# revdotcom/paper_accurate_fast_cheap

Hardware: AMD Instinct MI355X
Metric: audio-sec/sec (1/RTF) GigaSpeech long-form encode (higher is better)
Workload: dtype f32+bf16-slot

## Files before the change

include/pafc_encoder_ops.h:

```cpp
#ifndef PAFC_ENCODER_OPS_H
#define PAFC_ENCODER_OPS_H

#include "pafc_wkv6.h"

#ifdef __cplusplus
extern "C" {
#endif

int pafc_dwconv1d_cl(int dtype, int B, int T_in, int C, int K, int left_pad, int T_out, const void *x,
                     const void *w, const void *bias, void *y, int glu, const int32_t *lens,
                     pafc_stream_t stream);

int pafc_dwconv1d_cl_ex(int dtype, int B, int T_in, int C, int K, int left_pad, int T_out, const void *x, long ldx,
                        const void *w, const void *bias, void *y, int act, const int32_t *lens, pafc_stream_t stream);

int pafc_dwconv1d_cl_ln_silu(int dtype, int B, int T_in, int C, int K, int left_pad, int T_out, const void *x, long ldx,
                             const void *w, const void *bias, const void *gamma, const void *beta, float eps, void *y,
                             const int32_t *lens, pafc_stream_t stream);

size_t pafc_dwconv1d_cl_wgrad_workspace_bytes(int B, int T_out, int C, int K);
int pafc_dwconv1d_cl_wgrad(int dtype, int B, int T_in, int C, int K, int left_pad, int T_out, const void *x, long ldx,
                           const void *dy, float *dw, float *dbias, void *workspace, size_t workspace_bytes,
                           pafc_stream_t stream);

// ... 148 lines not shown

int pafc_mamba2_scan_skip_bf16(int B, int L, int H, const void *xbc, long ldx, const float *dt, const float *log_a,
                               const float *D, void *y_bf16, int reverse, int chunk_len, void *workspace,
                               size_t workspace_bytes, pafc_stream_t stream);
int pafc_mamba2_gate_norm(int dtype, long rows, int d_inner, const void *y, const void *z, long ld_z,
                          const void *norm_weight, float eps, void *out, pafc_stream_t stream);

int pafc_mamba2_scan_state(int B, int L, int H, const void *xbc, long ldx, const float *dt, const float *log_a, const float *D,
                           float *y_f32, void *y_bf16, const float *s_in, float *s_out, int reverse, int chunk_len,
                           void *workspace, size_t workspace_bytes, pafc_stream_t stream);

size_t pafc_mamba2_scan_bwd_workspace_bytes(int B, int L, int H, int chunk_len);
int pafc_mamba2_scan_backward(int B, int L, int H, const void *xbc, long ldx, const float *dt, const float *log_a,
                              const float *gy, void *g_xbc, long ldg, float *g_dt, float *g_la, int reverse, int chunk_len,
                              void *workspace, size_t workspace_bytes, pafc_stream_t stream);

int pafc_gemm_bf16(long M, int N, int K, int batch, const void *A, long lda, long strideA, const void *W, long ldw,
                   long strideW, const void *bias, long strideBias, const void *residual, long ldr, long strideR,
                   void *out, long ldo, long strideO, float alpha, int act, pafc_stream_t stream);
int pafc_gemm_bf16_glu_half(long M, int N, int K, int batch);
int pafc_conv3x3s2_nhwc_bf16_ph(int B, int T1, int F1, int Ci, int Co, const void *in, const void *w_tap_co_ci, const void *bias,
                                void *out, int relu, int tile_m, pafc_stream_t stream);
int pafc_gemm_bf16_ph(long M, int N, int K, int batch, const void *A, long lda, long strideA, const void *W, long ldw,
                      long strideW, const void *bias, long strideBias, const void *residual, long ldr, long strideR,
                      void *out, long ldo, long strideO, float alpha, int act, int tile_n, int tile_m, pafc_stream_t stream);
int pafc_gemm_ph_ex(long M, int N, int K, int batch, const void *A, long lda, long strideA, int a_split, const void *W, long ldw,
                    long strideW, const void *bias, long strideBias, const void *residual, int res_kind, long ldr, long strideR,
                    void *out, int out_kind, long ldo, long lo_off, long strideO, float alpha, int act, int tile_m,
                    pafc_stream_t stream);
int pafc_gemm_ph_ex2(long M, int N, int K, int batch, const void *A, long lda, long strideA, int a_split, int a_plane_block,
                     const void *W, long ldw, long strideW, const void *bias, long strideBias, const void *residual, int res_kind,
                     long ldr, long strideR, void *out, int out_kind, long ldo, long lo_off, long strideO, float alpha, int act,
                     int tile_m, pafc_stream_t stream);
int pafc_conv3x3s2_nhwc_split_ph(int B, int T1, int F1, int Ci, int Co, const void *in_planes, const void *w3_tap_co_3ci,
                                 const float *bias, void *out_planes, int relu, int tile_m, pafc_stream_t stream);

int pafc_residual_dropout(int backward, int dtype_x, int dtype_y, long n, const void *x, const void *y, void *out, float scale,
                          float p, unsigned long long seed, unsigned long long offset, pafc_stream_t stream);
int pafc_silu_dropout(int backward, int dtype, long n, const void *h, const void *dout, void *out, float p,
                      unsigned long long seed, unsigned long long offset, pafc_stream_t stream);

int pafc_multi_transpose_bf16(const void *table, int n, int total_tiles, pafc_stream_t stream);
int pafc_multi_cast_bf16(const void *table, int n, int total_chunks, pafc_stream_t stream);

int pafc_rows_gather(const long *table, const long *table_dev, int n, const int *idx, const int *offs, int m, int S,
                     pafc_stream_t stream);
int pafc_rows_scatter(const long *table, const long *table_dev, int n, const int *idx, int m, int S, pafc_stream_t stream);

#ifdef __cplusplus
}
#endif
#endif
```

paper_accurate_fast_cheap_amd/_lib.py:

```python
import ctypes
import os
from ctypes import c_float, c_int, c_long, c_size_t, c_ulonglong, c_void_p

import torch

_HERE = os.path.dirname(os.path.abspath(__file__))
SO_PATH = os.path.join(_HERE, "libpafc_hip.so")

PAFC_F32, PAFC_BF16 = 0, 1
_ERRORS = {
    -1: "null pointer", -2: "bad dims (B, T, C, H must be positive and C == H * 64)", -3: "head size must be 64",
    -4: "workspace too small", -5: "kernel launch failed", -6: "unsupported dtype", -7: "unsupported",
    -8: "r, k, v, w, y must be 16-byte aligned",
}


class PafcError(RuntimeError):
    pass


_lib = None


def lib():
# ... 60 lines not shown
    "pafc_conv3x3s2_nhwc_f32split": (I, [I, I, I, I, I, P, P, P, P, P, P, I, P]),
    "pafc_gemm_tn_workspace_bytes": (Z, [G, I, I]),
    "pafc_gemm_tn_bf16": (I, [G, I, I, P, G, P, G, P, P, I, P, Z, P]),
    "pafc_gemm_tn_batched_workspace_bytes": (Z, [G, I, I, I]),
    "pafc_gemm_tn_bf16_batched": (I, [G, I, I, I, P, G, G, P, G, G, P, P, I, P, Z, P]),
    "pafc_gemm_bf16_f32out": (I, [G, I, I, P, G, I, P, G, P, P, G, P, I, G, G, F, I, P, Z, P]),
    "pafc_gemm_bf16_f32out_pb": (I, [G, I, I, P, G, I, I, P, G, P, P, G, P, I, G, G, F, I, P, Z, P]),
    "pafc_gemm_bf16_f32out_workspace_bytes": (Z, [G, I, I, I]),
    "pafc_ctc_loss_workspace_bytes": (Z, [I, I, I]),
    "pafc_ctc_loss_forward": (I, [I, I, I, I, P, G, P, P, I, P, I, I, P, P, Z, P]),
    "pafc_ctc_loss_backward": (I, [I, I, I, I, P, G, P, P, I, P, I, I, P, P, F, P, G, P, Z, P]),
    "pafc_rnnt_joint_loss_workspace_bytes": (Z, [I, I, I, G, G, P, I]),
    "pafc_rnnt_joint_loss_forward": (I, [I, I, I, I, I, P, G, G, P, G, G, P, P, P, P, P, I, I, G, P, P, Z, P]),
    "pafc_rnnt_joint_loss_backward": (I, [I, I, I, I, I, P, G, G, P, G, G, P, P, P, P, P, I, I, G, P, G, P, F, I, P, P, P, P,
        P, Z, P, Z, P]),
    "pafc_gemm_f32": (I, [G, I, I, I, P, G, G, P, G, G, P, G, P, G, G, P, G, G, F, I, P]),
    "pafc_mamba2_prep": (I, [I, I, I, I, P, P, G, P, P, P, P, P, P, P, P, P]),
    "pafc_mamba2_finish": (I, [I, I, I, I, P, P, P, P, G, P, G, P, P, P, F, I, P, P]),
    "pafc_mamba2_scan_chunk_len": (I, [I, I, I]),
    "pafc_mamba2_scan_workspace_bytes": (Z, [I, I, I, I]),
    "pafc_mamba2_scan": (I, [I, I, I, P, G, P, P, P, I, P, Z, P]),
    "pafc_mamba2_scan_dir": (I, [I, I, I, P, G, P, P, P, I, I, P, Z, P]),
    "pafc_mamba2_scan_skip_bf16": (I, [I, I, I, P, G, P, P, P, P, I, I, P, Z, P]),
    "pafc_mamba2_gate_norm": (I, [I, G, I, P, P, G, P, F, P, P]),
    "pafc_mamba2_scan_state": (I, [I, I, I, P, G, P, P, P, P, P, P, P, I, I, P, Z, P]),
    "pafc_mamba2_scan_bwd_workspace_bytes": (Z, [I, I, I, I]),
    "pafc_mamba2_scan_backward": (I, [I, I, I, P, G, P, P, P, P, G, P, P, I, I, P, Z, P]),
    "pafc_gemm_bf16": (I, [G, I, I, I, P, G, G, P, G, G, P, G, P, G, G, P, G, G, F, I, P]),
    "pafc_gemm_bf16_glu_half": (I, [G, I, I, I]),
    "pafc_conv3x3s2_nhwc_bf16_ph": (I, [I, I, I, I, I, P, P, P, P, I, I, P]),
    "pafc_gemm_bf16_ph": (I, [G, I, I, I, P, G, G, P, G, G, P, G, P, G, G, P, G, G, F, I, I, I, P]),
    "pafc_gemm_ph_ex": (I, [G, I, I, I, P, G, G, I, P, G, G, P, G, P, I, G, G, P, I, G, G, G, F, I, I, P]),
    "pafc_gemm_ph_ex2": (I, [G, I, I, I, P, G, G, I, I, P, G, G, P, G, P, I, G, G, P, I, G, G, G, F, I, I, P]),
    "pafc_conv3x3s2_nhwc_split_ph": (I, [I, I, I, I, I, P, P, P, P, I, I, P]),
    "pafc_residual_dropout": (I, [I, I, I, G, P, P, P, F, F, U, U, P]),
    "pafc_silu_dropout": (I, [I, I, G, P, P, P, F, U, U, P]),
    "pafc_multi_transpose_bf16": (I, [P, I, I, P]),
    "pafc_multi_cast_bf16": (I, [P, I, I, P]),
    "pafc_rows_gather": (I, [P, P, I, P, P, I, I, P]),
    "pafc_rows_scatter": (I, [P, P, I, P, I, I, P]),
    "pafc_fbank_num_frames": (G, [G]),
    "pafc_fbank_tables_cols": (I, []),
    "pafc_fbank_f32": (I, [P, G, P, P, P, P, P, I, P, F, F, P, P]),
    "pafc_fbank_batch": (I, [P, G, P, I, G, P, P, P, P, P, I, P, F, F, P, I, P, P]),
    "pafc_fbank_stream_plan": (I, [I, G, P, P]),
    "pafc_fbank_stream": (I, [P, I, P, G, G, I, P, P, P, P, P, I, F, F, P, I, G, G, P]),
    "pafc_fbank_stream_rows": (I, [P, I, P, P, I, P, G, G, P, P, P, P, P, I, F, F, P, I, I, P]),
    "pafc_ctc_greedy": (I, [I, I, I, I, P, P, I, P, P, P, P, P]),
    "pafc_log_softmax_rows": (I, [I, G, I, P, P, P]),
    "pafc_ctc_prefix_beam_workspace_bytes": (Z, [I, I, I]),
    "pafc_ctc_prefix_beam_search": (I, [I, I, I, P, P, P, I, I, P, P, P, P, Z, P]),
    "pafc_ctc_prefix_beam_ex_workspace_bytes": (Z, [I, I, I]),
    "pafc_ctc_prefix_beam_search_ex": (I, [I, I, I, P, P, P, I, I, P, P, P, P, P, P, Z, P]),
    "pafc_ctc_beam_stream_workspace_bytes": (Z, [I, I, I, I]),
    "pafc_ctc_beam_stream_reset": (I, [I, I, I, I, P, P, Z, P]),
    "pafc_ctc_beam_stream_feed": (I, [I, I, I, P, P, P, I, I, I, P, I, P, Z, P]),
    "pafc_ctc_beam_stream_drain": (I, [I, I, I, P, I, P, Z, P, I, P, P, P, P, P, P, I, P, P, P]),
    "pafc_ctc_greedy_stream_workspace_bytes": (Z, [I]),
    "pafc_ctc_greedy_stream_reset": (I, [I, P, P, Z, P]),
    "pafc_ctc_greedy_stream": (I, [I, I, I, I, P, P, I, P, Z, P, P, P, P, P]),
    "pafc_ctc_align_workspace_bytes": (Z, [I, I, I]),
    "pafc_ctc_align": (I, [I, I, I, I, P, G, P, P, I, P, I, P, Z, P, P, P, I, P, P, P]),
    "pafc_rnnt_beam_workspace_bytes": (Z, [I, I, I]),
    "pafc_rnnt_beam_init": (I, [I, I, I, I, P, Z, P, P, P]),
    "pafc_rnnt_beam_step": (I, [I, I, I, I, I, P, P, P, P, P, Z, P, P, P]),
    "pafc_rnnt_beam_finish": (I, [I, I, I, P, Z, P, P, P, P]),
# ... 79 lines not shown
```

paper_accurate_fast_cheap_amd/csrc/gemm_bf16.hip:

```cpp
#include <stdio.h>
#include <stdlib.h>

#include "pafc_common.h"
#include "../../include/pafc_encoder_ops.h"

namespace pafc {
namespace {

constexpr int GBM = 128, GBN = 128, GBK = 64;
typedef float f32x4g __attribute__((ext_vector_type(4)));
typedef __bf16 bf16x8g __attribute__((ext_vector_type(8)));

struct GemmParams {
    const bf16_t *A, *W, *bias, *res;
    bf16_t *out;
    long M;
    int N, K;
    long lda, ldw, ldo, ldr;
    long sA, sW, sO, sB, sR;
    float alpha;
    int act;
    int mtiles, ntiles;
    int nk1, K1;
    int pb_sh;
// ... 294 lines not shown
                *reinterpret_cast<uint4 *>(Oz + m * p.ldo + n0 + c8) = *reinterpret_cast<const uint4 *>(O + row * LDO + c8);
        }
    }
}

}
}

extern "C" int pafc_gemm_bf16_ph(long M, int N, int K, int batch, const void *A, long lda, long strideA, const void *W, long ldw,
                                 long strideW, const void *bias, long strideBias, const void *residual, long ldr, long strideR,
                                 void *out, long ldo, long strideO, float alpha, int act, int tile_n, int tile_m,
                                 pafc_stream_t stream);

static int ph_tile_m(long M, int N, int K, int batch, int act, bool has_residual) {
    if (N % 8 || K % 128 || N < 256) return 0;
    if (act == 4 && N % 256) return 0;
    if (has_residual && act != 0) return 0;
    const int cus = pafc::device_cus();
    const long nt = (N + 255) / 256;
    static const long min_fill = [] { const char *e = getenv("PAFC_PH_MIN_FILL"); return e ? atol(e) : 0L; }();
    if (min_fill > 0) {
        if (((M + 255) / 256) * nt * batch * 100 < (long)cus * min_fill) return 0;
    } else if (((M + 127) / 128) * ((N + 127) / 128) * batch <= 2L * cus) {
        return 0;
    }
    long best_cost = -1;
    int best = 0;
    for (int tm = 256; tm >= 192; tm -= 64) {
        const long tiles = ((M + tm - 1) / tm) * nt * batch;
        const long cost = ((tiles + cus - 1) / cus) * (tm + 64);
        if (best_cost < 0 || cost < best_cost) { best_cost = cost; best = tm; }
    }
    return best;
}

extern "C" int pafc_gemm_bf16_glu_half(long M, int N, int K, int batch) { return ph_tile_m(M, N, K, batch, 4, false) ? 32 : 64; }

extern "C" int pafc_gemm_bf16(long M, int N, int K, int batch, const void *A, long lda, long strideA, const void *W,
                              long ldw, long strideW, const void *bias, long strideBias, const void *residual, long ldr,
                              long strideR, void *out, long ldo, long strideO, float alpha, int act,
                              pafc_stream_t stream) {
    if (!A || !W || !out) return PAFC_ERR_NULL_POINTER;
    if (M <= 0 || N <= 0 || K <= 0 || batch <= 0 || batch > 65535) return PAFC_ERR_BAD_DIMS;
    if (N % 8 || K % pafc::GBK) return PAFC_ERR_UNSUPPORTED;
    if (act < 0 || act > 4) return PAFC_ERR_UNSUPPORTED;
    if (const int tm = ph_tile_m(M, N, K, batch, act, residual != nullptr)) {
        const int rc = pafc_gemm_bf16_ph(M, N, K, batch, A, lda, strideA, W, ldw, strideW, bias, strideBias, residual, ldr, strideR,
                                         out, ldo, strideO, alpha, act, 256, tm, stream);
        if (rc != PAFC_ERR_UNSUPPORTED) return rc;
        if (act == 4) return PAFC_ERR_UNSUPPORTED;
    }
    const bool glu = act == 4;
    if (glu && (N % pafc::GBN || residual)) return PAFC_ERR_UNSUPPORTED;
    if (lda < K || ldw < K || ldo < (glu ? N / 2 : N) || (residual && ldr < N)) return PAFC_ERR_BAD_DIMS;
    if ((lda | ldw | ldo | strideA | strideW | strideO) % 8 || (residual && ((ldr | strideR) % 8))) return PAFC_ERR_ALIGNMENT;
    if ((((uintptr_t)A | (uintptr_t)W | (uintptr_t)out | (uintptr_t)residual) & 15) != 0) return PAFC_ERR_ALIGNMENT;
    pafc::GemmParams p{};
    p.A = (const pafc::bf16_t *)A; p.W = (const pafc::bf16_t *)W; p.bias = (const pafc::bf16_t *)bias;
    p.res = (const pafc::bf16_t *)residual; p.out = (pafc::bf16_t *)out;
    p.M = M; p.N = N; p.K = K;
    p.lda = lda; p.ldw = ldw; p.ldo = ldo; p.ldr = ldr;
    p.sA = strideA; p.sW = strideW; p.sO = strideO; p.sB = strideBias; p.sR = strideR;
    p.alpha = alpha; p.act = act;
    const long cus = pafc::device_cus();
    auto tiles = [&](int bm, int bn) { return ((M + bm - 1) / bm) * ((N + bn - 1) / bn) * (long)batch; };
    int bm = 128, bn = 128;
// ... 190 lines not shown
```

paper_accurate_fast_cheap_amd/csrc/gemm_ph.hip:

```cpp
#include <climits>
#include <cstdlib>
#include <cstring>
#include <type_traits>

#include "pafc_common.h"
#include "../../include/pafc_encoder_ops.h"

namespace pafc {
namespace {

typedef float f32x4p __attribute__((ext_vector_type(4)));
typedef __bf16 bf16x8p __attribute__((ext_vector_type(8)));
typedef unsigned u32x4p __attribute__((ext_vector_type(4)));

struct PhParams {
    const bf16_t *A, *W;
    const void *bias;
    const void *res;
    void *out;
    long M;
    int N, K;
    long lda, ldw, ldo, ldr;
    long sA, sW, sO, sB, sR;
    float alpha;
// ... 26 lines not shown
                                             uniform_off, 0, 0);
}
__device__ __forceinline__ __amdgpu_buffer_rsrc_t make_rsrc(const void *base, long bytes) {
    return __builtin_amdgcn_make_buffer_rsrc(const_cast<void *>(base), 0, (int)(bytes > 0x7fffffffL ? 0x7fffffffL : bytes), 0x00020000);
}

typedef float f32x2p __attribute__((ext_vector_type(2)));
typedef __bf16 bf16x2p __attribute__((ext_vector_type(2)));
__device__ __forceinline__ uint32_t pack_bf16(float lo, float hi) {
    return __builtin_bit_cast(uint32_t, __builtin_convertvector(f32x2p{lo, hi}, bf16x2p));
}

template <int ACT>
__device__ __forceinline__ float act_apply(float v) {
    if constexpr (ACT == 1) return v * __builtin_amdgcn_rcpf(1.f + __expf(-v));
    if constexpr (ACT == 2) return 1.f - 2.f * __builtin_amdgcn_rcpf(__expf(2.f * v) + 1.f);
    if constexpr (ACT == 3) return fmaxf(v, 0.f);
    return v;
}

#ifndef PH_ST_AUX
#define PH_ST_AUX 0
#endif
#define PH_WAIT(N) asm volatile("s_waitcnt vmcnt(" #N ")" ::: "memory")
template <int N>
__device__ __forceinline__ void wait_vm() {
    static_assert(N >= 0 && N < 64, "vmcnt is a 6-bit counter");
    asm volatile("s_waitcnt vmcnt(%0)" ::"n"(N) : "memory");
}

constexpr int PBN = 256, PBK = 64;
constexpr unsigned PH_OOB = 0xC0000000u;

template <bool GLU, int ACT, int RES, int OUT, bool CONV = false, int LNF = 0, bool SPL = false>
__global__ __launch_bounds__(512, 2) void gemm_ph_kernel(const PhParams p) {
    constexpr int BN = PBN;
    constexpr int UA = 128 * 128;
    constexpr int UB = (BN / 2) * 128;
    constexpr int STEP = 2 * UA + 2 * UB;
    constexpr int OFF_A0 = 0, OFF_A1 = UA, OFF_B0 = 2 * UA, OFF_B1 = 2 * UA + UB;
    constexpr int TN = 2;
    constexpr int DA = UA / 8192;
    constexpr int DB = UB / 8192;
    constexpr int OSZ = OUT == 1 ? 4 : 2;
    constexpr bool BIASF32 = OUT != 0;
    constexpr int NST = 8 * (GLU ? 1 : 2) * (OUT == 0 ? 1 : 2) + (LNF == 2 ? 8 : 0);
    static_assert(LNF == 0 || (OUT == 0 && !CONV), "LayerNorm folding: bf16 GEMMs");
    static_assert(!SPL || LNF == 0, "shared-fragment split operands: not with a folded LayerNorm");
    static_assert(LNF != 1 || (RES == 0 && (GLU || ACT == 1)), "LNF 1: the w_1 (SiLU) / pointwise_conv1 (GLU) projections");
    static_assert(LNF != 2 || RES == 1, "LNF 2: a residual GEMM");
    static_assert(!(GLU && (ACT != 0 || RES != 0)), "GLU excludes an activation and a residual");
    static_assert(!(RES != 0 && ACT != 0), "the layer never pairs a residual with an activation");
    extern __shared__ __attribute__((aligned(1024))) unsigned char lds[];

    const int tid = threadIdx.x, lane = tid & 63;
    const int wave = __builtin_amdgcn_readfirstlane(tid >> 6);
    const int wr = wave >> 2, wc = wave & 3;
    const long nblk = (long)p.mtiles * p.ntiles;
    const long total = nblk * p.batch;
    const long per = total / 8;
    const int nt = SPL ? p.nsteps : p.K / PBK;

    auto pix_off = [&](long m) -> long {
        const long tf = (long)p.T2 * p.F2;
        const long bb = m / tf, rem = m - bb * tf;
        const long t2 = rem / p.F2, f2 = rem - t2 * p.F2;
        return (((bb * p.T1 + 2 * t2) * p.F1 + 2 * f2) * p.CiA) * 2;
    };

    struct Tile {
        long m0;
        int n0, z, vr;
        __amdgpu_buffer_rsrc_t Ar, Wr;
    };
    auto make_tile = [&](long t, Tile &T) {
        const bool real = t < total;
        long tt = real ? t : 0;
        if (tt < per * 8) tt = (tt % 8) * per + tt / 8;
        T.z = (int)(tt / nblk);
        const long bid = tt % nblk;
        const int mt0 = (int)(bid / p.ntiles), nt0 = (int)(bid % p.ntiles);
        T.m0 = (long)mt0 * p.tm;
        T.n0 = nt0 * BN;
        T.vr = (int)min((long)p.tm, p.M - T.m0);
        if constexpr (CONV) {
// ... 34 lines not shown
                const unsigned coff = SPL ? (unsigned)(16 * (sc & 3) + (sc >> 2) * p.w_lo) : (unsigned)(16 * sc);
                b_off[h][j] = (unsigned)((long)((u >> 5) * 64 + h * 32 + pc) * (CONV ? p.CiW : p.ldw) * 2) + coff;
            }
    };
    auto a_soff = [&](int kt) -> unsigned {
        if constexpr (SPL && !CONV) {
            const int blk = kt >> p.pb_shift, c = kt - (blk << p.pb_shift);
            return (unsigned)(blk * 2 * p.pb_bytes + c * 64);
        } else if constexpr (SPL) {
            const int tap = (kt * p.inv_spt) >> 16, kc = kt - tap * p.spt;
            const int dt = (tap * 11) >> 5, df = tap - 3 * dt;
            return (unsigned)(((dt * p.F1 + df) * p.CiA) * 2 + kc * 64);
        } else if constexpr (!CONV) {
            const int seg = (kt >= p.nk1) + (kt >= 2 * p.nk1);
            const int r = kt - seg * p.nk1;
            const int blk = r >> p.pb_shift, c = r - (blk << p.pb_shift);
            return (unsigned)(blk * 2 * p.pb_bytes + (seg == 1 ? p.pb_bytes : 0) + c * 128);
        } else {
            const int tap = (kt * p.inv_spt) >> 16, kc = kt - tap * p.spt;
            const int seg = (kc >= p.nk1) + (kc >= 2 * p.nk1), cc = kc - seg * p.nk1;
            const int dt = (tap * 11) >> 5, df = tap - 3 * dt;
            return (unsigned)(((dt * p.F1 + df) * p.CiA + (seg == 1 ? p.Ci : 0)) * 2 + cc * 128);
        }
    };
    auto w_soff = [&](int kt) -> unsigned {
        if constexpr (!CONV) return SPL ? kt * p.w_step : kt * 128;
        const int tap = (kt * p.inv_spt) >> 16, kc = kt - tap * p.spt;
        return (unsigned)(tap * p.N * p.CiW * 2 + kc * (SPL ? 64 : 128));
    };
    auto stage_a = [&](const Tile &T, int h, int buf, int kt) {
#ifdef PH_ABL_NODMA
        return;
#endif
#pragma unroll
        for (int j = 0; j < DA; ++j)
            dma16(T.Ar, a_off[h][j], a_soff(kt), lds + buf * STEP + (h ? OFF_A1 : OFF_A0) + (wave * DA + j) * 1024);
    };
    auto stage_b = [&](const Tile &T, int h, int buf, int kt) {
#ifdef PH_ABL_NODMA
        return;
#endif
#pragma unroll
        for (int j = 0; j < DB; ++j)
            dma16(T.Wr, b_off[h][j], w_soff(kt), lds + buf * STEP + (h ? OFF_B1 : OFF_B0) + (wave * DB + j) * 1024);
    };

    const int fr = lane & 15, kq = lane >> 4;
    const unsigned frag = fr * 128 + ((kq ^ (fr & 7)) * 16);
    const unsigned la = wr * (64 * 128) + frag;
    const unsigned lb = wc * (32 * 128) + frag;

    bf16x8p af[4][2], bf0[TN][2], bf1[TN][2];
    auto read_a = [&](int h, int buf) {
#ifdef PH_ABL_NOREAD
        return;
#endif
        const unsigned char *base = lds + buf * STEP + (h ? OFF_A1 : OFF_A0);
#pragma unroll
        for (int i = 0; i < 4; ++i) {
            af[i][0] = *reinterpret_cast<const bf16x8p *>(base + la + i * 2048);
            af[i][1] = *reinterpret_cast<const bf16x8p *>(base + (la ^ 64) + i * 2048);
        }
    };
    auto read_b = [&](int h, int buf, bf16x8p (&dst)[TN][2]) {
#ifdef PH_ABL_NOREAD
        return;
#endif
        const unsigned char *base = lds + buf * STEP + (h ? OFF_B1 : OFF_B0);
#pragma unroll
        for (int j = 0; j < TN; ++j) {
            dst[j][0] = *reinterpret_cast<const bf16x8p *>(base + lb + j * 2048);
            dst[j][1] = *reinterpret_cast<const bf16x8p *>(base + (lb ^ 64) + j * 2048);
        }
    };
// ... 341 lines not shown
                        }
                    }
                    store8(o, live, row, col);
                }
                if constexpr (LNF == 2) { gst1[LNF == 2 ? g : 0] = live ? st1 : 0.f; gst2[LNF == 2 ? g : 0] = live ? st2 : 0.f; }
            }
            if constexpr (LNF == 1) row_norm(vn, nx_rstd, nx_nm);
        }
    }
    if constexpr (LNF == 2) {
        __builtin_amdgcn_sched_barrier(0);
#pragma unroll
        for (int g = 0; g < 8; ++g) { gst1[g] += __shfl_xor(gst1[g], 16, 64); gst2[g] += __shfl_xor(gst2[g], 16, 64); }
#pragma unroll
        for (int g = 0; g < 8; ++g) { gst1[g] += __shfl_xor(gst1[g], 32, 64); gst2[g] += __shfl_xor(gst2[g], 32, 64); }
        typedef unsigned u32x2p __attribute__((ext_vector_type(2)));
#pragma unroll
        for (int g = 0; g < 8; ++g) {
            const int row = wr * 128 + g * 16 + efr;
            const bool ok = ekq == 0 && row < cur.vr;
            const unsigned off = ok ? (unsigned)(row * 64 + ((cur.n0 >> 8) * 4 + wc) * 8) : PH_OOB;
            __builtin_amdgcn_raw_buffer_store_b64(u32x2p{__float_as_uint(gst1[g]), __float_as_uint(gst2[g])}, Sr, off, 0, 0);
        }
    }
    __builtin_amdgcn_sched_barrier(0);
    first = false;
    if constexpr (CONV) make_tile(t + gridDim.x, cur);
    else cur = nxt;
    PH_STAMP(53);
    }
    PH_WAIT(0);
}

template <bool GLU, int ACT, int RES, int OUT, bool CONV = false, int LNF = 0, bool SPL = false>
int launch_ph(const PhParams &p, int batch, hipStream_t s) {
    constexpr size_t lds = 2 * (2 * 128 * 128 + 2 * (PBN / 2) * 128) + 8 * 1024 + (LNF == 1 ? 8 * 1024 + 16 * 1024 : 0);
    auto kern = gemm_ph_kernel<GLU, ACT, RES, OUT, CONV, LNF, SPL>;
    static bool attr_set[64];
    int dev = 0;
    if (hipGetDevice(&dev) != hipSuccess) return PAFC_ERR_LAUNCH;
    if (dev < 0 || dev >= 64 || !attr_set[dev]) {
        if (hipFuncSetAttribute((const void *)kern, hipFuncAttributeMaxDynamicSharedMemorySize, (int)lds) != hipSuccess)
            return PAFC_ERR_LAUNCH;
        if (dev >= 0 && dev < 64) attr_set[dev] = true;
    }
    const int cus = device_cus();
    PhParams q = p;
    q.batch = batch;
    const long total = (long)p.mtiles * p.ntiles * batch;
    const long grid = total < cus ? total : cus;
    hipLaunchKernelGGL(kern, dim3((unsigned)grid), dim3(512), lds, s, q);
    return hipGetLastError() == hipSuccess ? PAFC_OK : PAFC_ERR_LAUNCH;
}

int g_split_walk = -1;
bool split_shared_fragments() {
    if (g_split_walk < 0) {
        const char *e = getenv("PAFC_SPLIT_WALK");
        g_split_walk = !(e && std::strcmp(e, "hilohi") == 0);
    }
    return g_split_walk != 0;
}

}
}

extern "C" int pafc_gemm_ph_ex(long M, int N, int K, int batch, const void *A, long lda, long strideA, int a_split, const void *W,
                               long ldw, long strideW, const void *bias, long strideBias, const void *residual, int res_kind,
                               long ldr, long strideR, void *out, int out_kind, long ldo, long lo_off, long strideO, float alpha,
                               int act, int tile_m, pafc_stream_t stream) {
// ... 156 lines not shown
    p.spt = p.CiW / 64;
    p.inv_spt = (65536 + p.spt - 1) / p.spt;
    for (int kt = 0; kt < p.K / 64 + 2; ++kt)
        if (((kt * p.inv_spt) >> 16) != kt / p.spt) return PAFC_ERR_UNSUPPORTED;
    p.T1 = T1; p.F1 = F1; p.T2 = T2; p.F2 = F2;
    p.in_bytes = (long)B * T1 * F1 * p.CiA * 2;
    p.tm = tile_m;
    p.mtiles = (int)((M + tile_m - 1) / tile_m);
    p.ntiles = (Co + 255) / 256;
    hipStream_t s = (hipStream_t)stream;
    if (split && pafc::split_shared_fragments()) {
        p.spt = Ci / 32;
        p.inv_spt = (65536 + p.spt - 1) / p.spt;
        p.nsteps = 9 * p.spt;
        for (int kt = 0; kt < p.nsteps + 2; ++kt)
            if (((kt * p.inv_spt) >> 16) != kt / p.spt) return PAFC_ERR_UNSUPPORTED;
        p.a_lo = Ci * 2;
        p.w_lo = 2 * Ci * 2;
        return relu ? pafc::launch_ph<false, 3, 0, 2, true, 0, true>(p, 1, s) : pafc::launch_ph<false, 0, 0, 2, true, 0, true>(p, 1, s);
    }
    if (split) return relu ? pafc::launch_ph<false, 3, 0, 2, true>(p, 1, s) : pafc::launch_ph<false, 0, 0, 2, true>(p, 1, s);
    return relu ? pafc::launch_ph<false, 3, 0, 0, true>(p, 1, s) : pafc::launch_ph<false, 0, 0, 0, true>(p, 1, s);
}

extern "C" int pafc_conv3x3s2_nhwc_bf16_ph(int B, int T1, int F1, int Ci, int Co, const void *in, const void *w_tap_co_ci,
                                           const void *bias, void *out, int relu, int tile_m, pafc_stream_t stream) {
    return conv_ph_launch(B, T1, F1, Ci, Co, in, w_tap_co_ci, bias, out, relu, tile_m, 0, stream);
}

extern "C" int pafc_conv3x3s2_nhwc_split_ph(int B, int T1, int F1, int Ci, int Co, const void *in_planes, const void *w3_tap_co_3ci,
                                            const float *bias, void *out_planes, int relu, int tile_m, pafc_stream_t stream) {
    return conv_ph_launch(B, T1, F1, Ci, Co, in_planes, w3_tap_co_3ci, bias, out_planes, relu, tile_m, 1, stream);
}
```

paper_accurate_fast_cheap_amd/hip_ops.py:

```python
import contextlib
import ctypes
import math
import os
import threading
import weakref
from typing import List, Optional

import torch

from . import _lib
from ._lib import c_int, c_void_p
from .utils import graph_step


DISPATCH = dict(skinny_max_rows=640, own_gemm_min_rows=1, lds_resident_min_rows=8192, split_gemm_min_rows=1024,
                ln_fold_min_rows=24576, dwconv_ln_silu_max_rows=24575, split_small_max_rows=8192, split_layers_min_rows=256)


def _load_dispatch():
    legacy = dict(skinny_max_rows="PAFC_SKINNY_MAX_ROWS", own_gemm_min_rows="PAFC_OWN_GEMM_MIN_ROWS",
                  lds_resident_min_rows="PAFC_LDS_RESIDENT_MIN_ROWS", split_gemm_min_rows="PAFC_SPLIT_GEMM_MIN_ROWS")
    for name, env in legacy.items():
        if os.environ.get(env):
            DISPATCH[name] = int(os.environ[env])
    for item in filter(None, os.environ.get("PAFC_DISPATCH", "").split(",")):
        name, _, value = item.partition("=")
        if name.strip() not in DISPATCH:
            raise ValueError(f"PAFC_DISPATCH: unknown threshold {name!r} (known: {sorted(DISPATCH)})")
        DISPATCH[name.strip()] = int(value)


_load_dispatch()


def train_gemms_own() -> bool:
    return os.environ.get("PAFC_TRAIN_OWN_GEMMS", "1") != "0"


def train_kernels_enabled() -> bool:
    import os
    return os.environ.get("PAFC_TRAIN_KERNELS", "1") != "0"


def depthwise_conv1d_cl(x: torch.Tensor, weight: torch.Tensor, bias: Optional[torch.Tensor], left_pad: int,
                        out_len: int, glu: bool = False, lens: Optional[torch.Tensor] = None) -> torch.Tensor:
    _lib.require_gpu(x, weight, bias, lens)
    B, T, Cx = x.shape
    C = Cx // 2 if glu else Cx
    K = weight.shape[-1]
# ... 1348 lines not shown
                                    int(ln_c or (K if csum is not None else N)),
                                    float(eps), _ph_tile_m(M, N, min_tm=128), _lib.stream_of(a))
    _lib.check(rc, "pafc_gemm_bf16_ph_ln")
    return out


def split_planes(x: torch.Tensor, triple: bool = False) -> torch.Tensor:
    _lib.require_gpu(x)
    if x.dtype != torch.float32 or x.stride(-1) != 1:
        raise _lib.PafcError("split_planes: contiguous fp32 input")
    K = x.shape[-1]
    rows = x.numel() // K
    out = torch.empty(x.shape[:-1] + ((3 if triple else 2) * K,), dtype=torch.bfloat16, device=x.device)
    L = _lib.lib()
    _lib.check(L.pafc_split_planes(rows, K, _lib.ptr(x), K, _lib.ptr(out), out.shape[-1], K, int(triple), _lib.stream_of(x)),
               "pafc_split_planes")
    return out


def _ph_tile_m(M: int, N: int, batch: int = 1, min_tm: int = 64) -> int:
    cus = torch.cuda.get_device_properties(torch.cuda.current_device()).multi_processor_count
    nt = (N + 255) // 256
    best = None
    for tm in (256, 192, 128, 64):
        if tm < min_tm:
            continue
        tiles = ((M + tm - 1) // tm) * nt * batch
        cost = ((tiles + cus - 1) // cus) * (tm + 64)
        if best is None or cost < best[0]:
            best = (cost, tm)
    return best[1]


def gemm_ph_ex(a: torch.Tensor, w: torch.Tensor, bias: Optional[torch.Tensor] = None, act: str = "none", alpha: float = 1.0,
               residual: Optional[torch.Tensor] = None, out: Optional[torch.Tensor] = None, a_split: bool = False,
               out_kind: str = "bf16", tile_m: int = 0, a_plane_block: int = 0) -> torch.Tensor:
    _lib.require_gpu(bias)
    for t in (a, w, residual, out):
        if t is not None and (not t.is_cuda or t.stride(-1) != 1):
            raise _lib.PafcError("gemm_ph_ex: GPU tensors with unit stride in the last dimension")
    if a.dtype != torch.bfloat16 or w.dtype != torch.bfloat16 or a.dim() != 2 or w.dim() != 2:
        raise _lib.PafcError("gemm_ph_ex: a and w are 2-d bf16 (planes of fp32 operands with a_split)")
    M = a.shape[0]
    N = w.shape[0]
    K = w.shape[1] // 3 if a_split else w.shape[1]
    if a.shape[1] != (2 * K if a_split else K) or (a_split and w.shape[1] != 3 * K):
        raise _lib.PafcError("gemm_ph_ex: a (M, K) x w (N, K); split: a (M, 2K) x w (N, 3K)")
    No = N // 2 if act == "glu" else N
    kinds = {"bf16": (0, torch.bfloat16, No), "f32": (1, torch.float32, No), "planes": (2, torch.bfloat16, 2 * No)}
    ok, odt, ocols = kinds[out_kind]
    if out is None:
        out = torch.empty((M, ocols), dtype=odt, device=a.device)
    if out.dtype != odt or tuple(out.shape) != (M, ocols):
        raise _lib.PafcError("gemm_ph_ex: out must be (M, N) in the output form's dtype ((M, 2N) bf16 for planes)")
    rk = 0
    if residual is not None:
        rk = 1 if residual.dtype == torch.bfloat16 else 2
        if tuple(residual.shape) != (M, N) or residual.dtype != (torch.bfloat16 if ok == 0 else torch.float32) or ok == 2:
            raise _lib.PafcError("gemm_ph_ex: residual (M, N) in the output dtype (bf16 / fp32), not with planes")
    if bias is not None and (bias.dtype != (torch.bfloat16 if ok == 0 else torch.float32) or bias.numel() != N):
        raise _lib.PafcError("gemm_ph_ex: bias (N) bf16 for a bf16 output, fp32 otherwise")
    L = _lib.lib()
    from .profiling import op_timer
    pb_ok = not a_plane_block or (a_split and a_plane_block >= 64 and a_plane_block & (a_plane_block - 1) == 0 and K % a_plane_block == 0)
    if (M <= _SPLIT_SMALL_MAX_ROWS and M * N <= _SPLIT_SMALL_MAX_OUT and ok != 0 and act in ("none", "silu", "tanh", "relu")
            and pb_ok and not tile_m and K % 64 == 0):
        nws = L.pafc_gemm_bf16_f32out_workspace_bytes(M, N, K, int(a_split))
        ws = torch.empty(nws, dtype=torch.uint8, device=a.device) if nws else None
        with op_timer("gemm%ss_%dx%d" % ("3" if a_split else "", K, N), sample=12, flops=2.0 * M * N * K * (3 if a_split else 1)):
            rc = L.pafc_gemm_bf16_f32out_pb(M, N, K, _lib.ptr(a), a.stride(0), int(a_split), int(a_plane_block), _lib.ptr(w), w.stride(0),
                                            _lib.ptr(bias), _lib.ptr(residual), residual.stride(0) if residual is not None else 0,
                                            _lib.ptr(out), ok, out.stride(0), No if ok == 2 else 0, float(alpha), _ACTS[act], _lib.ptr(ws),
                                            nws, _lib.stream_of(a))
        _lib.check(rc, "pafc_gemm_bf16_f32out")
        return out
    with op_timer("gemm%s_%dx%d" % ("3" if a_split else "", K, N), sample=12, flops=2.0 * M * N * K * (3 if a_split else 1)):
        rc = L.pafc_gemm_ph_ex2(M, N, K, 1, _lib.ptr(a), a.stride(0), 0, int(a_split), int(a_plane_block), _lib.ptr(w), w.stride(0), 0,
                                _lib.ptr(bias), 0,
                               _lib.ptr(residual), rk, residual.stride(0) if residual is not None else 0, 0, _lib.ptr(out), ok,
                               out.stride(0), No if ok == 2 else 0, 0, float(alpha), _ACTS[act], int(tile_m or _ph_tile_m(M, N)),
                               _lib.stream_of(a))
    _lib.check(rc, "pafc_gemm_ph_ex")
    return out


_SPLIT_SMALL_MAX_ROWS = DISPATCH["split_small_max_rows"]
_SPLIT_SMALL_MAX_OUT = 1 << 22


def wkv6_single_chunk(B: int, T: int, C: int, H: int) -> bool:
    return _lib.lib().pafc_wkv6_pick_chunk_len(B, T, C, H, 1) >= T


def _check_prev(prev: Optional[torch.Tensor], x: torch.Tensor):
    if prev is not None and (prev.dtype != x.dtype or prev.numel() != x.shape[0] * x.shape[2] or not prev.is_contiguous()
                             or prev.device != x.device):
        raise _lib.PafcError("tmix: prev must be a contiguous (B, C) tensor of x's dtype on x's device")


def tmix_shift_mix(x: torch.Tensor, maa_x0: torch.Tensor, maa_x1: Optional[torch.Tensor], reverse0: bool = False,
                   prev: Optional[torch.Tensor] = None):
    _lib.require_gpu(x, maa_x0, maa_x1, prev)
    _check_prev(prev, x)
    B, T, C = x.shape
    ndir = 2 if maa_x1 is not None else 1
    out = torch.empty((ndir, B, T, C), dtype=x.dtype, device=x.device)
    rc = _lib.lib().pafc_tmix_shift_mix_prev(_lib.dtype_code(x.dtype), B, T, C, ndir, int(reverse0), _lib.ptr(x),
# ... 1327 lines not shown
```

Baseline: 46260.

## Split-K the partial last wave of split-operand fp32 GEMMs

Adds a tail-wave split-K path for split-plane GEMMs with fp32 output. The full waves of 256x256 tiles run through the existing kernel, and the leftover rows run with the K dimension cut into two slices. Each slice writes fp32 partials to a workspace, and a fixup kernel sums them and applies bias, alpha and residual. This aims to fill idle CUs during the last partial wave, at the cost of an extra launch, workspace traffic, and a different summation order.

After: 46720 (median of 6 runs). +1.0%, better.

```diff
diff --git a/include/pafc_encoder_ops.h b/include/pafc_encoder_ops.h
--- a/include/pafc_encoder_ops.h
+++ b/include/pafc_encoder_ops.h
@@ -204,6 +204,11 @@
                      const void *W, long ldw, long strideW, const void *bias, long strideBias, const void *residual, int res_kind,
                      long ldr, long strideR, void *out, int out_kind, long ldo, long lo_off, long strideO, float alpha, int act,
                      int tile_m, pafc_stream_t stream);
+int pafc_gemm_ph_ktail(long M, int N, int K, int batch, const void *A, long lda, long strideA, int a_split, int a_plane_block,
+                       const void *W, long ldw, long strideW, const void *bias, long strideBias, const void *residual, int res_kind,
+                       long ldr, long strideR, void *out, int out_kind, long ldo, long lo_off, long strideO, float alpha, int act,
+                       int tile_m, void *workspace, size_t workspace_bytes, long split_row, int kslices, pafc_stream_t stream);
+int pafc_gemm_ph_ktail_plan(long M, int N, int K, int batch, int cus, int min_k, long *split_row);
 int pafc_conv3x3s2_nhwc_split_ph(int B, int T1, int F1, int Ci, int Co, const void *in_planes, const void *w3_tap_co_3ci,
                                  const float *bias, void *out_planes, int relu, int tile_m, pafc_stream_t stream);
 
diff --git a/paper_accurate_fast_cheap_amd/_lib.py b/paper_accurate_fast_cheap_amd/_lib.py
--- a/paper_accurate_fast_cheap_amd/_lib.py
+++ b/paper_accurate_fast_cheap_amd/_lib.py
@@ -116,6 +116,8 @@
     "pafc_gemm_bf16_ph": (I, [G, I, I, I, P, G, G, P, G, G, P, G, P, G, G, P, G, G, F, I, I, I, P]),
     "pafc_gemm_ph_ex": (I, [G, I, I, I, P, G, G, I, P, G, G, P, G, P, I, G, G, P, I, G, G, G, F, I, I, P]),
     "pafc_gemm_ph_ex2": (I, [G, I, I, I, P, G, G, I, I, P, G, G, P, G, P, I, G, G, P, I, G, G, G, F, I, I, P]),
+    "pafc_gemm_ph_ktail": (I, [G, I, I, I, P, G, G, I, I, P, G, G, P, G, P, I, G, G, P, I, G, G, G, F, I, I, P, Z, G, I, P]),
+    "pafc_gemm_ph_ktail_plan": (I, [G, I, I, I, I, I, P]),
     "pafc_conv3x3s2_nhwc_split_ph": (I, [I, I, I, I, I, P, P, P, P, I, I, P]),
     "pafc_residual_dropout": (I, [I, I, I, G, P, P, P, F, F, U, U, P]),
     "pafc_silu_dropout": (I, [I, I, G, P, P, P, F, U, U, P]),
diff --git a/paper_accurate_fast_cheap_amd/csrc/gemm_bf16.hip b/paper_accurate_fast_cheap_amd/csrc/gemm_bf16.hip
--- a/paper_accurate_fast_cheap_amd/csrc/gemm_bf16.hip
+++ b/paper_accurate_fast_cheap_amd/csrc/gemm_bf16.hip
@@ -350,6 +350,18 @@
         if (best_cost < 0 || cost < best_cost) { best_cost = cost; best = tm; }
     }
     return best;
+}
+
+extern "C" int pafc_gemm_ph_ktail_plan(long M, int N, int K, int batch, int cus, int min_k, long *split_row) {
+    if (split_row) *split_row = 0;
+    if (M <= 0 || N <= 0 || K <= 0 || batch != 1 || !split_row) return 0;
+    if (cus <= 0) cus = pafc::device_cus();
+    const long ntiles = (N + 255) / 256, tiles = ((M + 255) / 256) * ntiles;
+    const long full = tiles / cus * cus, tail = tiles - full;
+    if (full <= 0 || tail <= 0 || 2 * tail > cus || full % ntiles) return 0;
+    if (K % 128 || K < min_k) return 0;
+    *split_row = full / ntiles * 256;
+    return 2;
 }
 
 extern "C" int pafc_gemm_bf16_glu_half(long M, int N, int K, int batch) { return ph_tile_m(M, N, K, batch, 4, false) ? 32 : 64; }
diff --git a/paper_accurate_fast_cheap_amd/csrc/gemm_ph.hip b/paper_accurate_fast_cheap_amd/csrc/gemm_ph.hip
--- a/paper_accurate_fast_cheap_amd/csrc/gemm_ph.hip
+++ b/paper_accurate_fast_cheap_amd/csrc/gemm_ph.hip
@@ -82,7 +82,7 @@
 constexpr int PBN = 256, PBK = 64;
 constexpr unsigned PH_OOB = 0xC0000000u;
 
-template <bool GLU, int ACT, int RES, int OUT, bool CONV = false, int LNF = 0, bool SPL = false>
+template <bool GLU, int ACT, int RES, int OUT, bool CONV = false, int LNF = 0, bool SPL = false, bool KSL = false>
 __global__ __launch_bounds__(512, 2) void gemm_ph_kernel(const PhParams p) {
     constexpr int BN = PBN;
     constexpr int UA = 128 * 128;
@@ -101,6 +101,7 @@
     static_assert(LNF != 2 || RES == 1, "LNF 2: a residual GEMM");
     static_assert(!(GLU && (ACT != 0 || RES != 0)), "GLU excludes an activation and a residual");
     static_assert(!(RES != 0 && ACT != 0), "the layer never pairs a residual with an activation");
+    static_assert(!KSL || (SPL && !CONV && !GLU && ACT == 0 && RES == 0 && OUT == 1), "K slices: fp32 partial products of split operands");
     extern __shared__ __attribute__((aligned(1024))) unsigned char lds[];
 
     const int tid = threadIdx.x, lane = tid & 63;
@@ -201,6 +202,7 @@
 #ifdef PH_ABL_NODMA
         return;
 #endif
+        if constexpr (KSL) kt += T.z * nt;
 #pragma unroll
         for (int j = 0; j < DA; ++j)
             dma16(T.Ar, a_off[h][j], a_soff(kt), lds + buf * STEP + (h ? OFF_A1 : OFF_A0) + (wave * DA + j) * 1024);
@@ -209,6 +211,7 @@
 #ifdef PH_ABL_NODMA
         return;
 #endif
+        if constexpr (KSL) kt += T.z * nt;
 #pragma unroll
         for (int j = 0; j < DB; ++j)
             dma16(T.Wr, b_off[h][j], w_soff(kt), lds + buf * STEP + (h ? OFF_B1 : OFF_B0) + (wave * DB + j) * 1024);
@@ -616,10 +619,34 @@
     PH_WAIT(0);
 }
 
-template <bool GLU, int ACT, int RES, int OUT, bool CONV = false, int LNF = 0, bool SPL = false>
+__global__ __launch_bounds__(256) void gemm_ph_ktail_fixup_kernel(const float *__restrict__ part, long slab, int kslices,
+                                                                  const float *__restrict__ bias, const float *res, long ldr,
+                                                                  float *out, long ldo, long rows, int N, float alpha) {
+    const int nq = N >> 2;
+    const long total = rows * nq;
+    for (long i = (long)blockIdx.x * blockDim.x + threadIdx.x; i < total; i += (long)gridDim.x * blockDim.x) {
+        const long m = i / nq;
+        const int n = (int)(i - m * nq) << 2;
+        float4 acc = *reinterpret_cast<const float4 *>(part + m * N + n);
+        for (int z = 1; z < kslices; ++z) {
+            const float4 q = *reinterpret_cast<const float4 *>(part + z * slab + m * N + n);
+            acc.x += q.x; acc.y += q.y; acc.z += q.z; acc.w += q.w;
+        }
+        float4 b = make_float4(0.f, 0.f, 0.f, 0.f);
+        if (bias) b = *reinterpret_cast<const float4 *>(bias + n);
+        float4 o = make_float4(fmaf(acc.x, alpha, b.x), fmaf(acc.y, alpha, b.y), fmaf(acc.z, alpha, b.z), fmaf(acc.w, alpha, b.w));
+        if (res) {
+            const float4 r = *reinterpret_cast<const float4 *>(res + m * ldr + n);
+            o.x += r.x; o.y += r.y; o.z += r.z; o.w += r.w;
+        }
+        *reinterpret_cast<float4 *>(out + m * ldo + n) = o;
+    }
+}
+
+template <bool GLU, int ACT, int RES, int OUT, bool CONV = false, int LNF = 0, bool SPL = false, bool KSL = false>
 int launch_ph(const PhParams &p, int batch, hipStream_t s) {
     constexpr size_t lds = 2 * (2 * 128 * 128 + 2 * (PBN / 2) * 128) + 8 * 1024 + (LNF == 1 ? 8 * 1024 + 16 * 1024 : 0);
-    auto kern = gemm_ph_kernel<GLU, ACT, RES, OUT, CONV, LNF, SPL>;
+    auto kern = gemm_ph_kernel<GLU, ACT, RES, OUT, CONV, LNF, SPL, KSL>;
     static bool attr_set[64];
     int dev = 0;
     if (hipGetDevice(&dev) != hipSuccess) return PAFC_ERR_LAUNCH;
@@ -842,3 +869,70 @@
                                             const float *bias, void *out_planes, int relu, int tile_m, pafc_stream_t stream) {
     return conv_ph_launch(B, T1, F1, Ci, Co, in_planes, w3_tap_co_3ci, bias, out_planes, relu, tile_m, 1, stream);
 }
+
+extern "C" int pafc_gemm_ph_ktail(long M, int N, int K, int batch, const void *A, long lda, long strideA, int a_split,
+                                  int a_plane_block, const void *W, long ldw, long strideW, const void *bias, long strideBias,
+                                  const void *residual, int res_kind, long ldr, long strideR, void *out, int out_kind, long ldo,
+                                  long lo_off, long strideO, float alpha, int act, int tile_m, void *workspace,
+                                  size_t workspace_bytes, long split_row, int kslices, pafc_stream_t stream) {
+    if (!A || !W || !out || !workspace) return PAFC_ERR_NULL_POINTER;
+    if (M <= 0 || N <= 0 || K <= 0) return PAFC_ERR_BAD_DIMS;
+    if (act < 0 || act > 4 || out_kind < 0 || out_kind > 2 || res_kind < 0 || res_kind > 2) return PAFC_ERR_UNSUPPORTED;
+    if (!a_split || out_kind != 1 || act != 0 || batch != 1 || tile_m != 256 || kslices != 2) return PAFC_ERR_UNSUPPORTED;
+    if (!pafc::split_shared_fragments()) return PAFC_ERR_UNSUPPORTED;
+    if (!residual) res_kind = 0;
+    else if (res_kind == 0) return PAFC_ERR_BAD_DIMS;
+    else if (res_kind != 2) return PAFC_ERR_UNSUPPORTED;
+    if (split_row < 0 || split_row >= M || split_row % 256) return PAFC_ERR_BAD_DIMS;
+    if (K % (64 * kslices)) return PAFC_ERR_BAD_DIMS;
+    if (N % 8) return PAFC_ERR_UNSUPPORTED;
+    const long rows = M - split_row;
+    if (workspace_bytes < (size_t)kslices * (size_t)rows * (size_t)N * sizeof(float)) return PAFC_ERR_BAD_DIMS;
+    if (lda < 2 * (long)K || ldw < 3 * (long)K || (residual && ldr < N) || ldo < N) return PAFC_ERR_BAD_DIMS;
+    if ((lda | ldw) % 8 || ldo % 8 || (residual && ldr % 8)) return PAFC_ERR_ALIGNMENT;
+    if ((((uintptr_t)A | (uintptr_t)W | (uintptr_t)out | (uintptr_t)residual | (uintptr_t)bias | (uintptr_t)workspace) & 15) != 0)
+        return PAFC_ERR_ALIGNMENT;
+    if ((double)M * lda * 2 >= 2.0e9 || (double)N * ldw * 2 >= 2.0e9 || (double)2 * K * 2 + 64 >= 2.0e9) return PAFC_ERR_UNSUPPORTED;
+    if ((double)256 * ldo * 4 >= 2.0e9 || (residual && (double)256 * ldr * 4 >= 2.0e9)) return PAFC_ERR_UNSUPPORTED;
+    int pb_shift = 30;
+    long pb_bytes = (long)K * 2;
+    if (a_plane_block) {
+        int sh = 0;
+        while ((64 << sh) < a_plane_block) ++sh;
+        if ((64 << sh) != a_plane_block || K % a_plane_block) return PAFC_ERR_UNSUPPORTED;
+        pb_shift = sh + 1;
+        pb_bytes = (long)a_plane_block * 2;
+    }
+    hipStream_t s = (hipStream_t)stream;
+    if (split_row > 0) {
+        const int rc = pafc_gemm_ph_ex2(split_row, N, K, 1, A, lda, strideA, 1, a_plane_block, W, ldw, strideW, bias, strideBias,
+                                        residual, res_kind, ldr, strideR, out, 1, ldo, lo_off, strideO, alpha, 0, 256, stream);
+        if (rc != PAFC_OK) return rc;
+    }
+    pafc::PhParams p{};
+    p.A = (const pafc::bf16_t *)A + split_row * lda; p.W = (const pafc::bf16_t *)W; p.out = workspace;
+    p.M = rows; p.N = N; p.K = 3 * K;
+    p.lda = lda; p.ldw = ldw; p.ldo = N;
+    p.sO = rows * N;
+    p.alpha = 1.f;
+    p.nk1 = K / 64;
+    p.pb_shift = pb_shift;
+    p.pb_bytes = pb_bytes;
+    p.nsteps = K / 32 / kslices;
+    p.a_lo = (int)pb_bytes;
+    p.w_lo = 2 * K * 2;
+    p.w_step = 64;
+    p.tm = 256;
+    p.mtiles = (int)((rows + 255) / 256);
+    p.ntiles = (N + 255) / 256;
+    const int rc = pafc::launch_ph<false, 0, 0, 1, false, 0, true, true>(p, kslices, s);
+    if (rc != PAFC_OK) return rc;
+    const long quads = rows * (N / 4);
+    const long cap = (long)pafc::device_cus() * 32;
+    const long blocks = (quads + 255) / 256;
+    hipLaunchKernelGGL(pafc::gemm_ph_ktail_fixup_kernel, dim3((unsigned)(blocks < cap ? blocks : cap)), dim3(256), 0, s,
+                       (const float *)workspace, rows * N, kslices, (const float *)bias,
+                       residual ? (const float *)residual + split_row * ldr : nullptr, ldr, (float *)out + split_row * ldo, ldo, rows, N,
+                       alpha);
+    return hipGetLastError() == hipSuccess ? PAFC_OK : PAFC_ERR_LAUNCH;
+}
diff --git a/paper_accurate_fast_cheap_amd/hip_ops.py b/paper_accurate_fast_cheap_amd/hip_ops.py
--- a/paper_accurate_fast_cheap_amd/hip_ops.py
+++ b/paper_accurate_fast_cheap_amd/hip_ops.py
@@ -14,7 +14,8 @@
 
 
 DISPATCH = dict(skinny_max_rows=640, own_gemm_min_rows=1, lds_resident_min_rows=8192, split_gemm_min_rows=1024,
-                ln_fold_min_rows=24576, dwconv_ln_silu_max_rows=24575, split_small_max_rows=8192, split_layers_min_rows=256)
+                ln_fold_min_rows=24576, dwconv_ln_silu_max_rows=24575, split_small_max_rows=8192, split_layers_min_rows=256,
+                ktail_min_k=2048)
 
 
 def _load_dispatch():
@@ -1429,9 +1430,27 @@
     return best[1]
 
 
+def _ph_ktail_plan(M: int, N: int, K: int, cus: int, batch: int = 1, min_k: Optional[int] = None):
+    min_k = DISPATCH["ktail_min_k"] if min_k is None else min_k
+    if M <= 0 or N <= 0 or K <= 0 or batch != 1 or cus <= 0:
+        return None
+    ntiles = (N + 255) // 256
+    tiles = ((M + 255) // 256) * ntiles
+    full = tiles // cus * cus
+    tail = tiles - full
+    if full <= 0 or tail <= 0 or 2 * tail > cus or full % ntiles:
+        return None
+    if K % 128 or K < min_k:
+        return None
+    return full // ntiles * 256, 2
+
+
+_TAIL_AUTO = object()
+
+
 def gemm_ph_ex(a: torch.Tensor, w: torch.Tensor, bias: Optional[torch.Tensor] = None, act: str = "none", alpha: float = 1.0,
                residual: Optional[torch.Tensor] = None, out: Optional[torch.Tensor] = None, a_split: bool = False,
-               out_kind: str = "bf16", tile_m: int = 0, a_plane_block: int = 0) -> torch.Tensor:
+               out_kind: str = "bf16", tile_m: int = 0, a_plane_block: int = 0, tail_split=_TAIL_AUTO) -> torch.Tensor:
     _lib.require_gpu(bias)
     for t in (a, w, residual, out):
         if t is not None and (not t.is_cuda or t.stride(-1) != 1):
@@ -1461,7 +1480,7 @@
     from .profiling import op_timer
     pb_ok = not a_plane_block or (a_split and a_plane_block >= 64 and a_plane_block & (a_plane_block - 1) == 0 and K % a_plane_block == 0)
     if (M <= _SPLIT_SMALL_MAX_ROWS and M * N <= _SPLIT_SMALL_MAX_OUT and ok != 0 and act in ("none", "silu", "tanh", "relu")
-            and pb_ok and not tile_m and K % 64 == 0):
+            and pb_ok and not tile_m and K % 64 == 0 and (tail_split is _TAIL_AUTO or not tail_split)):
         nws = L.pafc_gemm_bf16_f32out_workspace_bytes(M, N, K, int(a_split))
         ws = torch.empty(nws, dtype=torch.uint8, device=a.device) if nws else None
         with op_timer("gemm%ss_%dx%d" % ("3" if a_split else "", K, N), sample=12, flops=2.0 * M * N * K * (3 if a_split else 1)):
@@ -1470,6 +1489,23 @@
                                             _lib.ptr(out), ok, out.stride(0), No if ok == 2 else 0, float(alpha), _ACTS[act], _lib.ptr(ws),
                                             nws, _lib.stream_of(a))
         _lib.check(rc, "pafc_gemm_bf16_f32out")
+        return out
+    if tail_split is _TAIL_AUTO:
+        tail_split = None
+        if a_split and ok == 1 and act == "none" and not tile_m and os.environ.get("PAFC_SPLIT_WALK") != "hilohi":
+            cus = torch.cuda.get_device_properties(a.device).multi_processor_count
+            tail_split = _ph_ktail_plan(M, N, K, cus)
+    if tail_split:
+        split_row, kslices = tail_split
+        nws = max(0, kslices * (M - split_row) * N * 4)
+        ws = torch.empty(max(nws, 16), dtype=torch.uint8, device=a.device)
+        with op_timer("gemm%s_%dx%d" % ("3" if a_split else "", K, N), sample=12, flops=2.0 * M * N * K * (3 if a_split else 1)):
+            rc = L.pafc_gemm_ph_ktail(M, N, K, 1, _lib.ptr(a), a.stride(0), 0, int(a_split), int(a_plane_block), _lib.ptr(w),
+                                      w.stride(0), 0, _lib.ptr(bias), 0, _lib.ptr(residual), rk,
+                                      residual.stride(0) if residual is not None else 0, 0, _lib.ptr(out), ok, out.stride(0),
+                                      No if ok == 2 else 0, 0, float(alpha), _ACTS[act], int(tile_m or 256), _lib.ptr(ws), nws,
+                                      int(split_row), int(kslices), _lib.stream_of(a))
+        _lib.check(rc, "pafc_gemm_ph_ktail")
         return out
     with op_timer("gemm%s_%dx%d" % ("3" if a_split else "", K, N), sample=12, flops=2.0 * M * N * K * (3 if a_split else 1)):
         rc = L.pafc_gemm_ph_ex2(M, N, K, 1, _lib.ptr(a), a.stride(0), 0, int(a_split), int(a_plane_block), _lib.ptr(w), w.stride(0), 0,
```
